# ladnlav/OFDM-course

Hardware: NVIDIA B200
Metric: OFDM symbols/s, full Task-5 RX chain (higher is better)
Workload: dtype f32

## Files before the change

### ofdm-course_b200/csrc/chain_rx4096.cu

```cuda
#include "interp.cuh"
#include "fft_reg.cuh"

#define FX_THREADS 256
#define XROW 288
#define XGRP 18
#define XBUF 4608
#define SLOT_ZERO (-2147483647 - 1)

const void* ofdm_upload_pilots(ofdm_ctx* ctx, const double* pv, size_t n_complex);
uint32_t ofdm_reg_to_prev(const uint8_t* reg);


__device__ __forceinline__ uint32_t ldg_once(const uint32_t* p) {
    uint32_t r;
    asm("ld.global.nc.L1::no_allocate.u32 %0, [%1];" : "=r"(r) : "l"(p));
    return r;
}
__device__ __forceinline__ void stg_once(uint32_t* p, uint32_t v) { asm volatile("st.global.L1::no_allocate.u32 [%0], %1;" ::"l"(p), "r"(v) : "memory"); }
__device__ __forceinline__ void stg_once(float2* p, float2 v) { asm volatile("st.global.L1::no_allocate.v2.f32 [%0], {%1, %2};" ::"l"(p), "f"(v.x), "f"(v.y) : "memory"); }

struct Fast4096Params {
    int Tg, S, SpF, Nc, Nd, Np, frame_words, frames, scramble, con_id;
    int txpf;
    int frame_bits, aligned;
    uint32_t prev0;
    const int32_t* slot;
    const float2* pilots;
    const float2* tw4096;
    float inv_sqrt10, two_a;
};

__device__ __forceinline__ uint32_t smem_u32(const void* p) { return (uint32_t)__cvta_generic_to_shared(p); }
__device__ __forceinline__ void mbar_init(uint64_t* bar, int count) {
    asm volatile("mbarrier.init.shared::cta.b64 [%0], %1;" ::"r"(smem_u32(bar)), "r"(count));
}
__device__ __forceinline__ void mbar_expect_tx(uint64_t* bar, uint32_t bytes) {
    asm volatile("mbarrier.arrive.expect_tx.shared::cta.b64 _, [%0], %1;" ::"r"(smem_u32(bar)), "r"(bytes) : "memory");
}
__device__ __forceinline__ void mbar_wait(uint64_t* bar, uint32_t parity) {
    asm volatile(
        "{\n\t.reg .pred p;\n\t"
        "WAIT_%=:\n\t"
        "mbarrier.try_wait.parity.shared::cta.b64 p, [%0], %1;\n\t"
        "@p bra DONE_%=;\n\t"
        "bra WAIT_%=;\n\t"
        "DONE_%=:\n\t}" ::"r"(smem_u32(bar)), "r"(parity) : "memory");
}
__device__ __forceinline__ void bulk_g2s(void* dst, const void* src, uint32_t bytes, uint64_t* bar) {
    asm volatile("cp.async.bulk.shared::cluster.global.mbarrier::complete_tx::bytes [%0], [%1], %2, [%3];" ::"r"(smem_u32(dst)), "l"(src),
                 "r"(bytes), "r"(smem_u32(bar))
                 : "memory");
}
__device__ __forceinline__ void bulk_prefetch_l2(const void* src, uint32_t bytes) {
    asm volatile("cp.async.bulk.prefetch.L2.global [%0], %1;" ::"l"(src), "r"(bytes) : "memory");
}
__device__ __forceinline__ void fence_proxy_async() { asm volatile("fence.proxy.async.shared::cta;" ::: "memory"); }

__host__ __device__ constexpr int mask_popc(int m) { int n = 0; for (int i = 0; i < 16; ++i) n += (m >> i) & 1; return n; }
__host__ __device__ constexpr int mask_perm(int m, int j) {
    int n = 0;
    for (int i = 0; i < 16; ++i) if ((m >> i) & 1) { if (n == j) return i; ++n; }
    for (int i = 0; i < 16; ++i) if (!((m >> i) & 1)) { if (n == j) return i; ++n; }
    return 0;
}
template <bool QAM16, bool NEAR, int MASK, bool SLIM>
__global__ void __launch_bounds__(FX_THREADS, SLIM ? 3 : 2) rx4096_kernel(Fast4096Params p, PlanDev<float> plan, DevConst<float> con, const float2* __restrict__ rx,
                                                               int64_t B, const uint32_t* __restrict__ txbits, uint32_t* __restrict__ outbits,
                                                               float2* __restrict__ Hout, unsigned long long* __restrict__ counts,
                                                               int32_t* __restrict__ err_stream, float near_eps, unsigned long long* __restrict__ next_stream) {
    extern __shared__ __align__(128) unsigned char smem_raw[];
    __shared__ __align__(8) uint64_t bars[2];
    float2* xb0 = (float2*)smem_raw;
    float2* Hinv = xb0 + (SLIM ? 1 : 2) * XBUF;
    float2* yk = Hinv + 1024;
    float2* dk = yk + plan.n_knots;
    int32_t* slot_s = (int32_t*)(dk + plan.n_knots);
    float2* pinv = (float2*)(slot_s + 1024);
    uint8_t* symidx = (uint8_t*)(pinv + p.Np);
    const int tid = threadIdx.x;
    const int bps = con.bps;
    for (int i = tid; i < 1024; i += FX_THREADS) slot_s[i] = p.slot[i];
    if (tid < 8) symidx[p.SpF * p.Nd + tid] = 0;
    for (int i = tid; i < p.Np; i += FX_THREADS) { float2 x = p.pilots[i]; float dd = x.x * x.x + x.y * x.y; pinv[i] = make_float2(x.x / dd, -x.y / dd); }

    constexpr int NTW = SLIM ? 4 : 16;
    float2 ta[NTW], tb[NTW];
    float2 ta4[SLIM ? 4 : 1], tb4[SLIM ? 4 : 1];
#pragma unroll
    for (int k1 = 0; k1 < NTW; ++k1) ta[k1] = p.tw4096[(tid * k1) & 4095];
    {
        const int n3 = tid & 15;
#pragma unroll
        for (int k2 = 0; k2 < NTW; ++k2) tb[k2] = p.tw4096[(16 * n3 * k2) & 4095];
        if (SLIM) {
#pragma unroll
            for (int d = 0; d < 4; ++d) { ta4[d] = p.tw4096[(4 * tid * d) & 4095]; tb4[d] = p.tw4096[(64 * n3 * d) & 4095]; }
        }
    }
    auto twa = [&](float2 x, int c, int d) -> float2 {
        if (SLIM) { if (c) x = cmul(x, ta[c]); if (d) x = cmul(x, ta4[d]); return x; }
        return (c + 4 * d) ? cmul(x, ta[SLIM ? 0 : c + 4 * d]) : x;
    };
    auto twb = [&](float2 x, int c, int d) -> float2 {
        if (SLIM) { if (c) x = cmul(x, tb[c]); if (d) x = cmul(x, tb4[d]); return x; }
        return (c + 4 * d) ? cmul(x, tb[SLIM ? 0 : c + 4 * d]) : x;
    };
    const int symlen = 4096 + p.Tg;
    const int64_t stream_words = (int64_t)p.frame_words * p.frames;
    const float two_a = p.two_a;
    const int64_t my_streams = (B - blockIdx.x + gridDim.x - 1) / gridDim.x;
    const int64_t n_items = my_streams * p.S;
    const int64_t stream_stride = (int64_t)p.S * symlen;
    const float2* rx0 = rx + (int64_t)blockIdx.x * stream_stride + p.Tg;
    const int k1c = (tid >> 6) + 4 * ((tid >> 3) & 3), k2c = ((tid >> 5) & 1) * 8 + (tid & 7);
    const int kq = k1c + 16 * k2c;
    const int k1b = mask_perm(MASK, tid >> 4);
    const bool b_idle = 2 * (tid >> 5) + 1 < mask_popc(MASK);
    uint32_t role01, role23;
    bool warp_data, warp_pil;
    {
        uint32_t r[4];
        bool anyd = false, anyp = false;
#pragma unroll
        for (int c = 0; c < 4; ++c) {
            const int sl = p.slot[kq + 256 * c];
            const bool in = kq + 256 * c < p.Nc;
            r[c] = (sl >= 0 && in) ? (uint32_t)sl : 0xFFFFu;
            anyd |= (sl >= 0 && in);
            anyp |= (sl < 0 && sl != SLOT_ZERO);
        }
        role01 = r[0] | (r[1] << 16); role23 = r[2] | (r[3] << 16);
        warp_data = __any_sync(0xffffffffu, anyd);
        warp_pil = __any_sync(0xffffffffu, anyp);
    }
    if (tid == 0) {
        mbar_init(&bars[0], 1);
        mbar_init(&bars[1], 1);
        asm volatile("fence.mbarrier_init.release.cluster;" ::: "memory");
    }
    __syncthreads();
    const float2* pf_ptr = rx0;
    int pf_s = 0;
    auto pf_advance = [&]() {
        if (++pf_s == p.S) { pf_s = 0; pf_ptr += (int64_t)gridDim.x * stream_stride - (int64_t)(p.S - 1) * symlen; }
        else pf_ptr += symlen;
    };
    if (tid == 0) {
        for (int i = 0; i < (SLIM ? 1 : 2) && i < n_items; ++i) {
            mbar_expect_tx(&bars[i], 32768u);
            bulk_g2s(xb0 + i * XBUF, pf_ptr, 32768u, &bars[i]);
            pf_advance();
        }
    }
    int errs = 0, nears = 0;
    int s = 0, sf = 0, f = 0;
    int sfNd = 0;
    int64_t b = blockIdx.x;
    uint32_t parity = 0;
    __shared__ long long s_bnext[2];
    int kpar = 0;
    const bool dyn = SLIM && next_stream != nullptr;
    int64_t bn = dyn ? B : b + gridDim.x;
    for (int64_t q = 0; dyn ? (b < B) : (q < n_items); ++q) {
        const int cur = SLIM ? 0 : (int)(q & 1);
        float2* X = xb0 + cur * XBUF;
        float2 v[16];
        if (dyn && s == 0 && tid == 0) { bn = (int64_t)gridDim.x + (int64_t)atomicAdd(next_stream, 1ull); s_bnext[kpar] = bn; }
        mbar_wait(&bars[cur], parity);
        parity ^= SLIM ? 1u : (uint32_t)cur;
#pragma unroll
        for (int n1 = 0; n1 < 16; ++n1) v[n1] = X[256 * n1 + tid];
        const bool pruned = MASK != 0 && s != 0;
        if (pruned) {
            fft16_steps12(v);
#pragma unroll
            for (int c = 0; c < 4; ++c)
                if (((MASK >> c) & 0x1111) != 0x1111) fft4(v[4 * c], v[4 * c + 1], v[4 * c + 2], v[4 * c + 3]);
#pragma unroll
            for (int c = 0; c < 4; ++c)
#pragma unroll
                for (int d = 0; d < 4; ++d) {
                    const int k1 = c + 4 * d;
                    if (!((MASK >> k1) & 1)) X[k1 * 256 + tid] = twa(v[4 * c + d], c, d);
                }
        } else {
            fft16(v);
#pragma unroll
            for (int c = 0; c < 4; ++c)
#pragma unroll
                for (int d = 0; d < 4; ++d) {
                    const int k1 = c + 4 * d;
                    X[k1 * 256 + tid] = twa(v[4 * c + d], c, d);
                }
        }
        __syncthreads();
        const bool b_active = !(pruned && b_idle);
        {
            float2* rp = X + k1b * 256 + (tid & 15);
            if (b_active) {
#pragma unroll
                for (int n2 = 0; n2 < 16; ++n2) v[n2] = rp[16 * n2];
            }
            __syncthreads();
            if (b_active) {
                fft16(v);
                float2* wp = X + k1b * XROW + (tid & 15);
#pragma unroll
                for (int c = 0; c < 4; ++c)
#pragma unroll
                    for (int d = 0; d < 4; ++d) {
                        const int k2 = c + 4 * d;
                        wp[XGRP * k2] = twb(v[4 * c + d], c, d);
                    }
            }
        }
        __syncthreads();
        {
            const float4* rp = reinterpret_cast<const float4*>(X + k1c * XROW + k2c * XGRP);
#pragma unroll
            for (int j = 0; j < 8; ++j) {
                const float4 w = rp[j];
                v[2 * j] = make_float2(w.x, w.y);
                v[2 * j + 1] = make_float2(w.z, w.w);
            }
        }
        __syncthreads();
        if (tid == 0 && (SLIM ? (s + 1 < p.S || bn < B) : (q + 2 < n_items))) {
            fence_proxy_async();
            mbar_expect_tx(&bars[cur], 32768u);
            if (SLIM) {
                const bool wrap = s + 1 == p.S;
                const float2* nxt = rx + (wrap ? bn : b) * stream_stride + (int64_t)(wrap ? 0 : s + 1) * symlen + p.Tg;
                bulk_g2s(X, nxt, 32768u, &bars[cur]);
                if (s + 2 < p.S) bulk_prefetch_l2(rx + b * stream_stride + (int64_t)(s + 2) * symlen + p.Tg, 32768u);
                else if (bn < B && s + 2 - p.S < p.S) bulk_prefetch_l2(rx + bn * stream_stride + (int64_t)(s + 2 - p.S) * symlen + p.Tg, 32768u);
            } else {
                bulk_g2s(X, pf_ptr, 32768u, &bars[cur]);
                pf_advance();
            }
        }
        if (SLIM && tid == 0 && txbits && p.txpf && sf == (p.SpF > 1 ? p.SpF - 2 : 0))
            bulk_prefetch_l2(txbits + b * stream_words + (int64_t)f * p.frame_words, (uint32_t)p.frame_words * 4u);
        uint32_t txw[4] = {0u, 0u, 0u, 0u};
        if (!SLIM && sf == p.SpF - 1 && txbits && p.aligned) {
            const uint32_t* tp = txbits + b * stream_words + (int64_t)f * p.frame_words + tid;
#pragma unroll
            for (int j = 0; j < 4; ++j) if (tid + FX_THREADS * j < p.frame_words) txw[j] = ldg_once(tp + FX_THREADS * j);
        }
        if (warp_data || s == 0) {
            fft16_steps12(v);
            float2 Y[4];
#pragma unroll
            for (int c = 0; c < 4; ++c) Y[c] = add2(add2(v[4 * c], v[4 * c + 1]), add2(v[4 * c + 2], v[4 * c + 3]));
            if (s == 0) {
                if (warp_pil) {
#pragma unroll
                    for (int c = 0; c < 4; ++c) {
                        const int sl = slot_s[kq + 256 * c];
                        if (sl < 0 && sl != SLOT_ZERO) { const int pi = -1 - sl; yk[plan.ext_lo + pi] = cmul(Y[c], pinv[pi]); }
                    }
                }
                __syncthreads();
                float2* Hrow = Hout ? Hout + b * p.Nc : nullptr;
                plan_apply_fn<float>(plan, yk, dk, [&](int q, float2 h) {
                    if (Hrow) stg_once(Hrow + q, h);
                    const float dd = h.x * h.x + h.y * h.y;
                    const int k1 = q & 15, k2 = (q >> 4) & 15;
                    Hinv[(((k1 & 3) << 6) | ((k2 >> 3) << 5) | ((k1 >> 2) << 3) | (k2 & 7)) + (q & ~255)] = make_float2(h.x / dd, -h.y / dd);
                });
                __syncthreads();
            }
            if (warp_data) {
                uint8_t* sp = symidx + sfNd;
#pragma unroll
                for (int c = 0; c < 4; ++c) {
                    const uint32_t dr = ((c < 2 ? role01 : role23) >> (16 * (c & 1))) & 0xFFFFu;
                    const float2 e = cmul(Y[c], Hinv[tid + 256 * c]);
                    float margin = 1.f;
                    uint32_t nib;
                    if (QAM16) nib = demap16_nib<NEAR>(e.x, e.y, two_a, &margin);
                    else nib = (uint32_t)nearest_idx(con, e.x, e.y, &margin);
                    asm volatile("{\n\t.reg .pred p;\n\tsetp.ne.u32 p, %0, 0xFFFF;\n\t@p st.shared.u8 [%1], %2;\n\t}" ::"r"(dr), "r"(smem_u32(sp) + dr), "r"(nib) : "memory");
                    if (NEAR && dr != 0xFFFFu && margin < near_eps) ++nears;
                }
            }
        }
        if (sf == p.SpF - 1 && !p.aligned) {
            __syncthreads();
            const int64_t stream_bits = (int64_t)p.frame_bits * p.frames;
            const int64_t fbase = b * stream_bits + (int64_t)f * p.frame_bits;
            auto packed = [&](int w) -> uint32_t {
                if (QAM16) {
                    const uint2 by = *reinterpret_cast<const uint2*>(symidx + 8 * w);
                    uint32_t lo = by.x | (by.x >> 4); lo = (lo & 0xFFu) | ((lo >> 8) & 0xFF00u);
                    uint32_t hi = by.y | (by.y >> 4); hi = (hi & 0xFFu) | ((hi >> 8) & 0xFF00u);
                    return lo | (hi << 16);
                }
                uint32_t word = 0;
                const int b0 = 32 * w, b1 = min(b0 + 32, p.frame_bits);
                for (int j = b0 / bps; j * bps < b1; ++j) {
                    int idx = symidx[j];
                    for (int i = 0; i < bps; ++i) {
                        int pos = j * bps + i;
                        if (pos >= b0 && pos < b1 && ((idx >> (bps - 1 - i)) & 1)) word |= 1u << (pos - b0);
                    }
                }
                return word;
            };
            for (int w = tid; w < p.frame_words; w += FX_THREADS) {
                const uint32_t cw = packed(w);
                uint32_t o = cw;
                if (p.scramble) { const uint32_t prev = w ? packed(w - 1) : p.prev0; o = cw ^ ((cw << 13) | (prev >> 19)) ^ ((cw << 14) | (prev >> 18)); }
                const int n = min(32, p.frame_bits - 32 * w);
                if (n < 32) o &= (1u << n) - 1u;
                if (txbits) errs += __popc(o ^ bits_get32(txbits, fbase + 32 * (int64_t)w, fbase + p.frame_bits));
                if (outbits) bits_put(outbits, fbase + 32 * (int64_t)w, n, o);
            }
            __syncthreads();
        } else if (sf == p.SpF - 1) {
            __syncthreads();
            const int64_t wbase = b * stream_words + (int64_t)f * p.frame_words;
            auto packed = [&](int w) -> uint32_t {
                if (QAM16) {
                    const uint2 by = *reinterpret_cast<const uint2*>(symidx + 8 * w);
                    uint32_t lo = by.x | (by.x >> 4); lo = (lo & 0xFFu) | ((lo >> 8) & 0xFF00u);
                    uint32_t hi = by.y | (by.y >> 4); hi = (hi & 0xFFu) | ((hi >> 8) & 0xFF00u);
                    return lo | (hi << 16);
                }
                uint32_t word = 0;
                const int b0 = 32 * w, b1 = b0 + 32;
                for (int j = b0 / bps; j * bps < b1; ++j) {
                    int idx = symidx[j];
                    for (int i = 0; i < bps; ++i) {
                        int pos = j * bps + i;
                        if (pos >= b0 && pos < b1 && ((idx >> (bps - 1 - i)) & 1)) word |= 1u << (pos - b0);
                    }
                }
                return word;
            };
#pragma unroll
            for (int j = 0; j < 4; ++j) {
                const int w = tid + FX_THREADS * j;
                if (w < p.frame_words) {
                    const uint32_t cw = packed(w);
                    uint32_t o = cw;
                    if (p.scramble) {
                        const uint32_t prev = w ? packed(w - 1) : p.prev0;
                        o = cw ^ ((cw << 13) | (prev >> 19)) ^ ((cw << 14) | (prev >> 18));
                    }
                    if (txbits) errs += __popc(o ^ (SLIM ? ldg_once(txbits + wbase + w) : txw[j]));
                    if (outbits) stg_once(outbits + wbase + w, o);
                }
            }
            for (int w = tid + 4 * FX_THREADS; w < p.frame_words; w += FX_THREADS) {
                const uint32_t cw = packed(w);
                uint32_t o = cw;
                if (p.scramble) { const uint32_t prev = packed(w - 1); o = cw ^ ((cw << 13) | (prev >> 19)) ^ ((cw << 14) | (prev >> 18)); }
                if (txbits) errs += __popc(o ^ txbits[wbase + w]);
                if (outbits) outbits[wbase + w] = o;
            }
        }
        sfNd += p.Nd;
        if (++sf == p.SpF) { sf = 0; sfNd = 0; ++f; }
        if (++s == p.S) {
            const int we = warp_sum(errs);
            if ((tid & 31) == 0 && we) {
                if (counts) atomicAdd(&counts[0], (unsigned long long)we);
                if (err_stream) atomicAdd(&err_stream[b], we);
            }
            if (NEAR) {
                const int wn = warp_sum(nears);
                if ((tid & 31) == 0 && wn && counts) atomicAdd(&counts[2], (unsigned long long)wn);
            }
            if (tid == 0 && counts) atomicAdd(&counts[1], (unsigned long long)((int64_t)p.frame_bits * p.frames));
            errs = 0; nears = 0; s = 0; sf = 0; sfNd = 0; f = 0;
            if (dyn) { b = s_bnext[kpar]; kpar ^= 1; } else { b += gridDim.x; bn = b + gridDim.x; }
        }
    }
}

int ofdm_rx_chain_fast4096(ofdm_ctx* ctx, const ofdm_link_params* lp, const void* rx, int64_t B, const uint32_t* tx_bits, uint32_t* out_bits,
                           void* H, int64_t* counts, int32_t* err_stream, double near_eps, bool* handled) {
    *handled = false;
    if (ctx->precision != OFDM_PREC_F32 || lp->Nfft != 4096 || lp->N_carrier > 1024 || lp->N_carrier < 2) return OFDM_OK;
    ConstTable ct = host_constellation(lp->constellation);
    if (ct.bps == 0 || lp->S <= 0 || lp->SpF <= 0 || lp->S % lp->SpF) return OFDM_OK;
    const int frame_bits = lp->SpF * lp->Nd * ct.bps;
    if (lp->Np < 2 || lp->Nd < 1) return OFDM_OK;
    if (getenv("OFDM_B200_NO_FAST")) return OFDM_OK;
    std::vector<int32_t> slot(1024, SLOT_ZERO);
    for (int i = 0; i < lp->Nd; ++i) { int c = lp->data_carriers_host[i]; if (c < 1 || c > lp->N_carrier) return OFDM_OK; slot[c - 1] = i; }
    for (int i = 0; i < lp->Np; ++i) {
        int c = lp->pilot_carriers_host[i];
        if (c < 1 || c > lp->N_carrier || (i && c <= lp->pilot_carriers_host[i - 1])) return OFDM_OK;
        slot[c - 1] = -1 - i;
    }
    const InterpPlan* pl = ctx_plan(ctx, lp->pilot_carriers_host, lp->Np, lp->N_carrier, nullptr, lp->N_carrier, OFDM_INTERP_SPLINE);
    REQUIRE(ctx, pl != nullptr, "plan construction failed");
    Fast4096Params p;
    p.Tg = lp->Tg; p.S = lp->S; p.SpF = lp->SpF; p.Nc = lp->N_carrier; p.Nd = lp->Nd; p.Np = lp->Np;
    p.frame_words = (frame_bits + 31) / 32; p.frames = lp->S / lp->SpF; p.scramble = lp->scramble; p.con_id = lp->constellation;
    p.frame_bits = frame_bits; p.aligned = frame_bits % 32 == 0;
    p.txpf = p.aligned && (p.frame_words & 3) == 0 && (((uintptr_t)tx_bits) & 15) == 0 && !getenv("OFDM_B200_NO_TXPF");
    p.prev0 = ofdm_reg_to_prev(lp->reg0_host);
    p.slot = (const int32_t*)ctx_blob(ctx, slot.data(), sizeof(int32_t) * 1024);
    p.pilots = (const float2*)ofdm_upload_pilots(ctx, lp->pilot_vals_host, lp->Np);
    p.tw4096 = (const float2*)ctx_twiddles(ctx, 4096);
    p.inv_sqrt10 = (float)ct.re[12];
    p.two_a = 2.f * p.inv_sqrt10;
    REQUIRE(ctx, p.slot && p.pilots && p.tw4096, "device upload failed");
    if (lp->Tg & 1) return OFDM_OK;
    if (((uintptr_t)rx) & 15) return OFDM_OK;
    size_t smem = sizeof(float2) * (2 * XBUF + 1024 + 2 * (size_t)pl->n_knots) + sizeof(int32_t) * 1024 +
                  (size_t)lp->SpF * lp->Nd + 8 + sizeof(float2) * (size_t)lp->Np + 32;
    if (smem > 110 * 1024) return OFDM_OK;
    const bool q16 = lp->constellation == OFDM_16QAM;
    const bool near = near_eps > 0.0;
    int dead = 0xFFFF;
    for (int k = 0; k < 1024; ++k) if (slot[k] >= 0) dead &= ~(1 << (k & 15));
    if (getenv("OFDM_B200_NO_PRUNE")) dead = 0;
    typedef void (*kern_t)(Fast4096Params, PlanDev<float>, DevConst<float>, const float2*, int64_t, const uint32_t*, uint32_t*, float2*, unsigned long long*,
                           int32_t*, float, unsigned long long*);
    kern_t kern;
    const size_t smem_slim = smem - sizeof(float2) * XBUF;
    const bool slim = getenv("OFDM_B200_NO_SLIM") == nullptr && smem_slim <= 74 * 1024;
    if (q16 && (dead & 0x1111) == 0x1111) {
        if (slim) kern = near ? rx4096_kernel<true, true, 0x1111, true> : rx4096_kernel<true, false, 0x1111, true>;
        else kern = near ? rx4096_kernel<true, true, 0x1111, false> : rx4096_kernel<true, false, 0x1111, false>;
    } else if (q16 && (dead & 0x0101) == 0x0101) {
        if (slim) kern = near ? rx4096_kernel<true, true, 0x0101, true> : rx4096_kernel<true, false, 0x0101, true>;
        else kern = near ? rx4096_kernel<true, true, 0x0101, false> : rx4096_kernel<true, false, 0x0101, false>;
    } else if (q16) {
        if (slim) kern = near ? rx4096_kernel<true, true, 0, true> : rx4096_kernel<true, false, 0, true>;
        else kern = near ? rx4096_kernel<true, true, 0, false> : rx4096_kernel<true, false, 0, false>;
    } else kern = near ? rx4096_kernel<false, true, 0, false> : rx4096_kernel<false, false, 0, false>;
    const bool use_slim = slim && q16;
    if (use_slim) smem = smem_slim;
    CUDA_TRY(ctx, cudaFuncSetAttribute(kern, cudaFuncAttributeMaxDynamicSharedMemorySize, (int)smem));
    int grid = (int)std::min<int64_t>(B, (int64_t)ctx->sm_count * (use_slim ? 3 : 2));
    if (err_stream) CUDA_TRY(ctx, cudaMemsetAsync(err_stream, 0, sizeof(int32_t) * B, ctx->stream));
    if (out_bits && !p.aligned) CUDA_TRY(ctx, cudaMemsetAsync(out_bits, 0, sizeof(uint32_t) * OFDM_BIT_WORDS(B * (int64_t)frame_bits * p.frames), ctx->stream));
    DevConst<float> con = make_devconst<float>(lp->constellation);
    PlanDev<float> pd = plan_dev<float>(pl);
    unsigned long long* sched = nullptr;
    if (use_slim && B > grid && !getenv("OFDM_B200_STATIC_STREAMS")) {
        CUDA_TRY(ctx, cudaMallocAsync((void**)&sched, sizeof(unsigned long long), ctx->stream));
        CUDA_TRY(ctx, cudaMemsetAsync(sched, 0, sizeof(unsigned long long), ctx->stream));
    }
    kern<<<grid, FX_THREADS, smem, ctx->stream>>>(p, pd, con, (const float2*)rx, B, tx_bits, out_bits, (float2*)H, (unsigned long long*)counts, err_stream,
                                                  (float)near_eps, sched);
    if (sched) cudaFreeAsync(sched, ctx->stream);
    LAUNCH_CHECK(ctx);
    *handled = true;
    return OFDM_OK;
}
```

Baseline: 116.1 million.

## Shrink SLIM kernel smem and registers to fit four CTAs per SM

For the SLIM variant, the slot table and pilot inverses move out of shared memory and are read from global via __ldg, recomputing the pilot inverse on demand. The knot buffers alias the symbol-index buffer, and Hinv is stored compactly when the pruning mask drops a quarter of the rows. Twiddle registers are cut by rebuilding power tables from fewer base twiddles each iteration, and the stream index is narrowed to int. Launch bounds rise to 4 CTAs per SM with the grid sized from the occupancy API. The goal is more resident CTAs to hide latency, at the cost of extra global loads, recomputed divisions and twiddle multiplies, and aliasing hazards between the knot and symbol buffers.

```diff
diff --git a/ofdm-course_b200/csrc/chain_rx4096.cu b/ofdm-course_b200/csrc/chain_rx4096.cu
--- a/ofdm-course_b200/csrc/chain_rx4096.cu
+++ b/ofdm-course_b200/csrc/chain_rx4096.cu
@@ -1,5 +1,7 @@
 #include "interp.cuh"
 #include "fft_reg.cuh"
+#include <climits>
+#include <type_traits>
 
 #define FX_THREADS 256
 #define XROW 288
@@ -64,45 +66,54 @@
     return 0;
 }
 template <bool QAM16, bool NEAR, int MASK, bool SLIM>
-__global__ void __launch_bounds__(FX_THREADS, SLIM ? 3 : 2) rx4096_kernel(Fast4096Params p, PlanDev<float> plan, DevConst<float> con, const float2* __restrict__ rx,
+__global__ void __launch_bounds__(FX_THREADS, SLIM ? 4 : 2) rx4096_kernel(Fast4096Params p, PlanDev<float> plan, DevConst<float> con, const float2* __restrict__ rx,
                                                                int64_t B, const uint32_t* __restrict__ txbits, uint32_t* __restrict__ outbits,
                                                                float2* __restrict__ Hout, unsigned long long* __restrict__ counts,
                                                                int32_t* __restrict__ err_stream, float near_eps, unsigned long long* __restrict__ next_stream) {
     extern __shared__ __align__(128) unsigned char smem_raw[];
     __shared__ __align__(8) uint64_t bars[2];
+    constexpr bool HCOMPACT = SLIM && MASK == 0x1111;
     float2* xb0 = (float2*)smem_raw;
     float2* Hinv = xb0 + (SLIM ? 1 : 2) * XBUF;
-    float2* yk = Hinv + 1024;
-    float2* dk = yk + plan.n_knots;
-    int32_t* slot_s = (int32_t*)(dk + plan.n_knots);
-    float2* pinv = (float2*)(slot_s + 1024);
-    uint8_t* symidx = (uint8_t*)(pinv + p.Np);
+    float2 *yk, *dk, *pinv = nullptr;
+    int32_t* slot_s = nullptr;
+    uint8_t* symidx;
+    if (SLIM) {
+        symidx = (uint8_t*)(Hinv + (HCOMPACT ? 768 : 1024));
+        yk = (float2*)symidx;
+        dk = yk + plan.n_knots;
+    } else {
+        yk = Hinv + 1024;
+        dk = yk + plan.n_knots;
+        slot_s = (int32_t*)(dk + plan.n_knots);
+        pinv = (float2*)(slot_s + 1024);
+        symidx = (uint8_t*)(pinv + p.Np);
+    }
     const int tid = threadIdx.x;
     const int bps = con.bps;
-    for (int i = tid; i < 1024; i += FX_THREADS) slot_s[i] = p.slot[i];
     if (tid < 8) symidx[p.SpF * p.Nd + tid] = 0;
-    for (int i = tid; i < p.Np; i += FX_THREADS) { float2 x = p.pilots[i]; float dd = x.x * x.x + x.y * x.y; pinv[i] = make_float2(x.x / dd, -x.y / dd); }
-
-    constexpr int NTW = SLIM ? 4 : 16;
-    float2 ta[NTW], tb[NTW];
-    float2 ta4[SLIM ? 4 : 1], tb4[SLIM ? 4 : 1];
-#pragma unroll
-    for (int k1 = 0; k1 < NTW; ++k1) ta[k1] = p.tw4096[(tid * k1) & 4095];
+    if (!SLIM) {
+        for (int i = tid; i < 1024; i += FX_THREADS) slot_s[i] = p.slot[i];
+        for (int i = tid; i < p.Np; i += FX_THREADS) { float2 x = p.pilots[i]; float dd = x.x * x.x + x.y * x.y; pinv[i] = make_float2(x.x / dd, -x.y / dd); }
+    }
+
+    constexpr int NTA = SLIM ? 4 : 16, NTB = SLIM ? 2 : 16;
+    float2 ta[NTA], tb[NTB];
+#pragma unroll
+    for (int k1 = 0; k1 < NTA; ++k1) ta[k1] = p.tw4096[(tid * k1) & 4095];
     {
         const int n3 = tid & 15;
 #pragma unroll
-        for (int k2 = 0; k2 < NTW; ++k2) tb[k2] = p.tw4096[(16 * n3 * k2) & 4095];
-        if (SLIM) {
-#pragma unroll
-            for (int d = 0; d < 4; ++d) { ta4[d] = p.tw4096[(4 * tid * d) & 4095]; tb4[d] = p.tw4096[(64 * n3 * d) & 4095]; }
-        }
-    }
-    auto twa = [&](float2 x, int c, int d) -> float2 {
-        if (SLIM) { if (c) x = cmul(x, ta[c]); if (d) x = cmul(x, ta4[d]); return x; }
+        for (int k2 = 0; k2 < NTB; ++k2) tb[k2] = p.tw4096[(16 * n3 * k2) & 4095];
+    }
+    auto powers = [](float2 x, float2* w) { w[1] = x; w[2] = cmul(x, x); w[3] = cmul(w[2], x); };
+    auto in_loop = [](float2 x) { asm volatile("" : "+f"(x.x), "+f"(x.y)); return x; };
+    auto twa = [&](float2 x, int c, int d, const float2* td) -> float2 {
+        if (SLIM) { if (c) x = cmul(x, ta[c]); if (d) x = cmul(x, td[d]); return x; }
         return (c + 4 * d) ? cmul(x, ta[SLIM ? 0 : c + 4 * d]) : x;
     };
-    auto twb = [&](float2 x, int c, int d) -> float2 {
-        if (SLIM) { if (c) x = cmul(x, tb[c]); if (d) x = cmul(x, tb4[d]); return x; }
+    auto twb = [&](float2 x, int c, int d, const float2* tc, const float2* td) -> float2 {
+        if (SLIM) { if (c) x = cmul(x, tc[c]); if (d) x = cmul(x, td[d]); return x; }
         return (c + 4 * d) ? cmul(x, tb[SLIM ? 0 : c + 4 * d]) : x;
     };
     const int symlen = 4096 + p.Tg;
@@ -155,42 +166,46 @@
     int errs = 0, nears = 0;
     int s = 0, sf = 0, f = 0;
     int sfNd = 0;
-    int64_t b = blockIdx.x;
+    auto frame = [&]() { return SLIM ? s / p.SpF : f; };
+    std::conditional_t<SLIM, int, int64_t> b = blockIdx.x;
     uint32_t parity = 0;
-    __shared__ long long s_bnext[2];
+    __shared__ int s_bnext[2];
     int kpar = 0;
     const bool dyn = SLIM && next_stream != nullptr;
-    int64_t bn = dyn ? B : b + gridDim.x;
-    for (int64_t q = 0; dyn ? (b < B) : (q < n_items); ++q) {
+    int64_t bn = b + gridDim.x;
+    for (int64_t q = 0; SLIM ? (b < B) : (q < n_items); ++q) {
         const int cur = SLIM ? 0 : (int)(q & 1);
         float2* X = xb0 + cur * XBUF;
         float2 v[16];
-        if (dyn && s == 0 && tid == 0) { bn = (int64_t)gridDim.x + (int64_t)atomicAdd(next_stream, 1ull); s_bnext[kpar] = bn; }
+        if (SLIM && s == 0 && tid == 0) s_bnext[kpar] = dyn ? (int)gridDim.x + (int)atomicAdd(next_stream, 1ull) : (int)b + (int)gridDim.x;
         mbar_wait(&bars[cur], parity);
         parity ^= SLIM ? 1u : (uint32_t)cur;
 #pragma unroll
         for (int n1 = 0; n1 < 16; ++n1) v[n1] = X[256 * n1 + tid];
         const bool pruned = MASK != 0 && s != 0;
+        float2 tc[4], td[4];
         if (pruned) {
             fft16_steps12(v);
 #pragma unroll
             for (int c = 0; c < 4; ++c)
                 if (((MASK >> c) & 0x1111) != 0x1111) fft4(v[4 * c], v[4 * c + 1], v[4 * c + 2], v[4 * c + 3]);
+            if (SLIM) { const float2 w2 = in_loop(ta[2]); powers(cmul(w2, w2), td); }
 #pragma unroll
             for (int c = 0; c < 4; ++c)
 #pragma unroll
                 for (int d = 0; d < 4; ++d) {
                     const int k1 = c + 4 * d;
-                    if (!((MASK >> k1) & 1)) X[k1 * 256 + tid] = twa(v[4 * c + d], c, d);
+                    if (!((MASK >> k1) & 1)) X[k1 * 256 + tid] = twa(v[4 * c + d], c, d, td);
                 }
         } else {
             fft16(v);
+            if (SLIM) { const float2 w2 = in_loop(ta[2]); powers(cmul(w2, w2), td); }
 #pragma unroll
             for (int c = 0; c < 4; ++c)
 #pragma unroll
                 for (int d = 0; d < 4; ++d) {
                     const int k1 = c + 4 * d;
-                    X[k1 * 256 + tid] = twa(v[4 * c + d], c, d);
+                    X[k1 * 256 + tid] = twa(v[4 * c + d], c, d, td);
                 }
         }
         __syncthreads();
@@ -200,22 +215,26 @@
             if (b_active) {
 #pragma unroll
                 for (int n2 = 0; n2 < 16; ++n2) v[n2] = rp[16 * n2];
+            } else if (SLIM) {
+#pragma unroll
+                for (int n2 = 0; n2 < 16; ++n2) v[n2] = make_float2(0.f, 0.f);
             }
             __syncthreads();
             if (b_active) {
                 fft16(v);
+                if (SLIM) { powers(in_loop(tb[1]), tc); powers(cmul(tc[2], tc[2]), td); }
                 float2* wp = X + k1b * XROW + (tid & 15);
 #pragma unroll
                 for (int c = 0; c < 4; ++c)
 #pragma unroll
                     for (int d = 0; d < 4; ++d) {
                         const int k2 = c + 4 * d;
-                        wp[XGRP * k2] = twb(v[4 * c + d], c, d);
+                        wp[XGRP * k2] = twb(v[4 * c + d], c, d, tc, td);
                     }
             }
         }
         __syncthreads();
-        {
+        if (!SLIM || warp_data || s == 0) {
             const float4* rp = reinterpret_cast<const float4*>(X + k1c * XROW + k2c * XGRP);
 #pragma unroll
             for (int j = 0; j < 8; ++j) {
@@ -223,8 +242,12 @@
                 v[2 * j] = make_float2(w.x, w.y);
                 v[2 * j + 1] = make_float2(w.z, w.w);
             }
+        } else {
+#pragma unroll
+            for (int j = 0; j < 16; ++j) v[j] = make_float2(0.f, 0.f);
         }
         __syncthreads();
+        if (SLIM && tid == 0) bn = s_bnext[kpar];
         if (tid == 0 && (SLIM ? (s + 1 < p.S || bn < B) : (q + 2 < n_items))) {
             fence_proxy_async();
             mbar_expect_tx(&bars[cur], 32768u);
@@ -240,7 +263,7 @@
             }
         }
         if (SLIM && tid == 0 && txbits && p.txpf && sf == (p.SpF > 1 ? p.SpF - 2 : 0))
-            bulk_prefetch_l2(txbits + b * stream_words + (int64_t)f * p.frame_words, (uint32_t)p.frame_words * 4u);
+            bulk_prefetch_l2(txbits + b * stream_words + (int64_t)frame() * p.frame_words, (uint32_t)p.frame_words * 4u);
         uint32_t txw[4] = {0u, 0u, 0u, 0u};
         if (!SLIM && sf == p.SpF - 1 && txbits && p.aligned) {
             const uint32_t* tp = txbits + b * stream_words + (int64_t)f * p.frame_words + tid;
@@ -256,26 +279,35 @@
                 if (warp_pil) {
 #pragma unroll
                     for (int c = 0; c < 4; ++c) {
-                        const int sl = slot_s[kq + 256 * c];
-                        if (sl < 0 && sl != SLOT_ZERO) { const int pi = -1 - sl; yk[plan.ext_lo + pi] = cmul(Y[c], pinv[pi]); }
+                        const int sl = SLIM ? __ldg(p.slot + kq + 256 * c) : slot_s[kq + 256 * c];
+                        if (sl < 0 && sl != SLOT_ZERO) {
+                            const int pi = -1 - sl;
+                            float2 pv;
+                            if (SLIM) { const float2 x = __ldg(p.pilots + pi); const float dd = x.x * x.x + x.y * x.y; pv = make_float2(x.x / dd, -x.y / dd); }
+                            else pv = pinv[pi];
+                            yk[plan.ext_lo + pi] = cmul(Y[c], pv);
+                        }
                     }
                 }
                 __syncthreads();
-                float2* Hrow = Hout ? Hout + b * p.Nc : nullptr;
+                float2* Hrow = Hout ? Hout + (int64_t)b * p.Nc : nullptr;
                 plan_apply_fn<float>(plan, yk, dk, [&](int q, float2 h) {
                     if (Hrow) stg_once(Hrow + q, h);
                     const float dd = h.x * h.x + h.y * h.y;
                     const int k1 = q & 15, k2 = (q >> 4) & 15;
-                    Hinv[(((k1 & 3) << 6) | ((k2 >> 3) << 5) | ((k1 >> 2) << 3) | (k2 & 7)) + (q & ~255)] = make_float2(h.x / dd, -h.y / dd);
+                    const int t = ((k1 & 3) << 6) | ((k2 >> 3) << 5) | ((k1 >> 2) << 3) | (k2 & 7);
+                    if (!HCOMPACT) Hinv[t + (q & ~255)] = make_float2(h.x / dd, -h.y / dd);
+                    else if (t >= 64) Hinv[t - 64 + 192 * (q >> 8)] = make_float2(h.x / dd, -h.y / dd);
                 });
                 __syncthreads();
+                if (SLIM && tid < 8) symidx[p.SpF * p.Nd + tid] = 0;
             }
             if (warp_data) {
-                uint8_t* sp = symidx + sfNd;
+                uint8_t* sp = symidx + (SLIM ? sf * p.Nd : sfNd);
 #pragma unroll
                 for (int c = 0; c < 4; ++c) {
                     const uint32_t dr = ((c < 2 ? role01 : role23) >> (16 * (c & 1))) & 0xFFFFu;
-                    const float2 e = cmul(Y[c], Hinv[tid + 256 * c]);
+                    const float2 e = cmul(Y[c], HCOMPACT ? Hinv[tid - 64 + 192 * c] : Hinv[tid + 256 * c]);
                     float margin = 1.f;
                     uint32_t nib;
                     if (QAM16) nib = demap16_nib<NEAR>(e.x, e.y, two_a, &margin);
@@ -288,7 +320,7 @@
         if (sf == p.SpF - 1 && !p.aligned) {
             __syncthreads();
             const int64_t stream_bits = (int64_t)p.frame_bits * p.frames;
-            const int64_t fbase = b * stream_bits + (int64_t)f * p.frame_bits;
+            const int64_t fbase = b * stream_bits + (int64_t)frame() * p.frame_bits;
             auto packed = [&](int w) -> uint32_t {
                 if (QAM16) {
                     const uint2 by = *reinterpret_cast<const uint2*>(symidx + 8 * w);
@@ -319,7 +351,7 @@
             __syncthreads();
         } else if (sf == p.SpF - 1) {
             __syncthreads();
-            const int64_t wbase = b * stream_words + (int64_t)f * p.frame_words;
+            const int64_t wbase = b * stream_words + (int64_t)frame() * p.frame_words;
             auto packed = [&](int w) -> uint32_t {
                 if (QAM16) {
                     const uint2 by = *reinterpret_cast<const uint2*>(symidx + 8 * w);
@@ -374,7 +406,7 @@
             }
             if (tid == 0 && counts) atomicAdd(&counts[1], (unsigned long long)((int64_t)p.frame_bits * p.frames));
             errs = 0; nears = 0; s = 0; sf = 0; sfNd = 0; f = 0;
-            if (dyn) { b = s_bnext[kpar]; kpar ^= 1; } else { b += gridDim.x; bn = b + gridDim.x; }
+            if (SLIM) { b = s_bnext[kpar]; kpar ^= 1; } else { b += gridDim.x; bn = b + gridDim.x; }
         }
     }
 }
@@ -422,8 +454,9 @@
     typedef void (*kern_t)(Fast4096Params, PlanDev<float>, DevConst<float>, const float2*, int64_t, const uint32_t*, uint32_t*, float2*, unsigned long long*,
                            int32_t*, float, unsigned long long*);
     kern_t kern;
-    const size_t smem_slim = smem - sizeof(float2) * XBUF;
-    const bool slim = getenv("OFDM_B200_NO_SLIM") == nullptr && smem_slim <= 74 * 1024;
+    const size_t smem_slim = sizeof(float2) * (XBUF + ((dead & 0x1111) == 0x1111 ? 768 : 1024)) +
+                             std::max((size_t)lp->SpF * lp->Nd + 8, 2 * sizeof(float2) * (size_t)pl->n_knots);
+    const bool slim = getenv("OFDM_B200_NO_SLIM") == nullptr && smem_slim <= 74 * 1024 && B <= INT_MAX / 2;
     if (q16 && (dead & 0x1111) == 0x1111) {
         if (slim) kern = near ? rx4096_kernel<true, true, 0x1111, true> : rx4096_kernel<true, false, 0x1111, true>;
         else kern = near ? rx4096_kernel<true, true, 0x1111, false> : rx4096_kernel<true, false, 0x1111, false>;
@@ -437,7 +470,12 @@
     const bool use_slim = slim && q16;
     if (use_slim) smem = smem_slim;
     CUDA_TRY(ctx, cudaFuncSetAttribute(kern, cudaFuncAttributeMaxDynamicSharedMemorySize, (int)smem));
-    int grid = (int)std::min<int64_t>(B, (int64_t)ctx->sm_count * (use_slim ? 3 : 2));
+    int per_sm = 2;
+    if (use_slim) {
+        CUDA_TRY(ctx, cudaOccupancyMaxActiveBlocksPerMultiprocessor(&per_sm, kern, FX_THREADS, smem));
+        REQUIRE(ctx, per_sm >= 3, "rx4096_kernel: fewer than three CTAs per SM");
+    }
+    int grid = (int)std::min<int64_t>(B, (int64_t)ctx->sm_count * per_sm);
     if (err_stream) CUDA_TRY(ctx, cudaMemsetAsync(err_stream, 0, sizeof(int32_t) * B, ctx->stream));
     if (out_bits && !p.aligned) CUDA_TRY(ctx, cudaMemsetAsync(out_bits, 0, sizeof(uint32_t) * OFDM_BIT_WORDS(B * (int64_t)frame_bits * p.frames), ctx->stream));
     DevConst<float> con = make_devconst<float>(lp->constellation);
```

New measurement: 119.7 million (median of 6 runs). 3.1% higher.
